# yanivw12/gs2mesh

Measured on AMD Instinct MI355X. Metric: stereo-pair renders/sec + TSDF Mvoxel-updates/sec, higher is better.
Workload: dtype f32

## Files before the change

gs2mesh_amd/csrc/tsdf_kernels.h:

```cpp
#pragma once
#include "tsdf_common.h"


GS2M_DEVICE void tsdf_cam_point(const TsdfFrame& f, float p0, float p1, float p2, float& pc0, float& pc1, float& pc2) {
    pc0 = f.E[0] * p0 + f.E[1] * p1 + f.E[2] * p2 + f.E[3] * 1.f;
    pc1 = f.E[4] * p0 + f.E[5] * p1 + f.E[6] * p2 + f.E[7] * 1.f;
    pc2 = f.E[8] * p0 + f.E[9] * p1 + f.E[10] * p2 + f.E[11] * 1.f;
}
GS2M_DEVICE void tsdf_z_step(const TsdfFrame& f, float& pc0, float& pc1, float& pc2) {
    pc0 += f.Es02;
    pc1 += f.Es12;
    pc2 += f.Es22;
}
GS2M_DEVICE int tsdf_project(const TsdfFrame& f, float pc0, float pc1, float pc2, int& u, int& v) {
    if (pc2 <= 0) return -1;
    const float u_f = pc0 * f.fx_f / pc2 + f.cx_f + 0.5f;
    const float v_f = pc1 * f.fy_f / pc2 + f.cy_f + 0.5f;
    if (!(u_f >= 0.0001f && u_f < f.safe_w && v_f >= 0.0001f && v_f < f.safe_h)) return -1;
    u = (int)u_f;
    v = (int)v_f;
    return v * f.W + u;
}
GS2M_DEVICE float tsdf_distance_multiplier(const TsdfFrame& f, int u, int v) {
    const float xx = (u - f.cx_f) * f.fx_inv_f;
    const float yy = (v - f.cy_f) * f.fy_inv_f;
    return sqrtf(xx * xx + yy * yy + 1.0f);
}
GS2M_DEVICE float tsdf_read_depth(const TsdfFrame& f, const float* __restrict__ depth, const unsigned char* __restrict__ mask, size_t pix) {
    float d = depth[pix];
    if (f.use_mask && mask[pix] == 0) d = d * 0.0f;
    return d;
}
GS2M_DEVICE float tsdf_convert_depth(const TsdfFrame& f, float d) {
    if (f.use_min && d < f.min_depth_f) d = 0.0f;
    if (f.depth_scale_f != 1.0f) d /= f.depth_scale_f;
    if (d >= f.depth_trunc_up_f) d = 0.0f;
    return d;
}
GS2M_DEVICE bool tsdf_decide(const TsdfFrame& f, float d, float zc, float mult, float& tnew) {
    const float sdf = (d - zc) * mult;
    tnew = fminf(1.0f, sdf * f.sdf_trunc_inv_f);
    return d > 0.0f && sdf > -f.sdf_trunc_f;
}
GS2M_DEVICE unsigned tsdf_gather_rgb(const unsigned char* __restrict__ color, int pix, int last_pix) {
    const unsigned char* c = color + 3 * (size_t)pix;
    return pix < last_pix ? gs2m_load_u32_unaligned(c) : ((unsigned)c[0] | ((unsigned)c[1] << 8) | ((unsigned)c[2] << 16));
}
GS2M_DEVICE void tsdf_update_mean(float& t, float& w, float tnew) {
    t = (t * w + tnew) / (w + 1.0f);
    w = w + 1.0f;
}
GS2M_DEVICE void tsdf_update_rgb(unsigned& c0, unsigned& c1, unsigned& c2, unsigned rgbp) {
    c0 += rgbp & 0xffu;
    c1 += (rgbp >> 8) & 0xffu;
    c2 += (rgbp >> 16) & 0xffu;
}
GS2M_DEVICE float tsdf_block_centres(const TsdfFrame& f, unsigned long long key, int tid, float* s_p0, float* s_p1) {
    int bx, by, bz;
    tsdf_unpack_key(key, bx, by, bz);
    const double ox = (double)bx * f.unit_length, oy = (double)by * f.unit_length, oz = (double)bz * f.unit_length;
    if (tid < 16) s_p0[tid] = (float)(f.half_voxel_length_f + f.voxel_length_f * tid + ox);
    else if (tid < 32) s_p1[tid - 16] = (float)(f.half_voxel_length_f + f.voxel_length_f * (tid - 16) + oy);
    return (float)(f.half_voxel_length_f + oz);
}

GS2M_DEVICE unsigned tsdf_find_or_insert(const TsdfVolume& V, unsigned long long key, int bx, int by, int bz) {
    const unsigned mask = V.hash_cap - 1u;
    unsigned h = tsdf_hash(key) & mask;
    for (unsigned probe = 0; probe < V.hash_cap; ++probe, h = (h + 1u) & mask) {
        unsigned long long k = V.hash_keys[h];
        if (k == key) return h;
        if (k == GS2M_TSDF_EMPTY) {
            const unsigned long long prev = atomicCAS(&V.hash_keys[h], GS2M_TSDF_EMPTY, key);
            if (prev == GS2M_TSDF_EMPTY) {
                const unsigned slot = atomicAdd(&V.counters[0], 1u);
                if (slot < V.max_blocks) {
                    V.block_keys[3 * (size_t)slot] = bx;
                    V.block_keys[3 * (size_t)slot + 1] = by;
                    V.block_keys[3 * (size_t)slot + 2] = bz;
                    V.hash_vals[h] = (int)slot;
                } else {
                    atomicOr(&V.counters[2], 1u);
                }
                return h;
            }
            if (prev == key) return h;
        }
    }
    atomicOr(&V.counters[2], 2u);
    return 0xffffffffu;
}

GS2M_DEVICE int tsdf_lookup(const TsdfVolume& V, unsigned long long key) {
    const unsigned mask = V.hash_cap - 1u;
    unsigned h = tsdf_hash(key) & mask;
    for (unsigned probe = 0; probe < V.hash_cap; ++probe, h = (h + 1u) & mask) {
        const unsigned long long k = V.hash_keys[h];
        if (k == key) return V.hash_vals[h];
        if (k == GS2M_TSDF_EMPTY) return -1;
    }
    return -1;
}

struct TouchStage {
    int lo[3][64];
    int hi[3][64];
};

GS2M_DEVICE int wave_min_i(int v) {
#pragma unroll
    for (int m = 32; m > 0; m >>= 1) {
        const int o = gs2m_shfl_xor(v, m);
        v = o < v ? o : v;
    }
    return v;
}
GS2M_DEVICE int wave_max_i(int v) {
#pragma unroll
    for (int m = 32; m > 0; m >>= 1) {
        const int o = gs2m_shfl_xor(v, m);
        v = o > v ? o : v;
    }
    return v;
}

GS2M_DEVICE void tsdf_touch_body(const TsdfVolume& V, const TsdfFrame& f, const float* __restrict__ depth,
                                 const unsigned char* __restrict__ mask, TouchStage* stage_all, int batch_bit) {
    const int lane = (int)(threadIdx.x & 63u);
    TouchStage* stg = &stage_all[threadIdx.x >> 6];
    const int idx = (int)(blockIdx.x * 256u + threadIdx.x);
    int lo[3] = {0x7fffffff, 0x7fffffff, 0x7fffffff}, hi[3] = {-0x7fffffff, -0x7fffffff, -0x7fffffff};
    bool valid = false;
    if (idx < f.nx * f.ny) {
        const int i = (idx / f.nx) * f.stride;
        const int j = (idx % f.nx) * f.stride;
        const float p = tsdf_convert_depth(f, tsdf_read_depth(f, depth, mask, (size_t)i * f.W + j));
        if (p > 0.0f) {
            valid = true;
            const double z = (double)p;
            const double x = (j - f.cx) * z / f.fx;
            const double y = (i - f.cy) * z / f.fy;
#pragma unroll
            for (int r = 0; r < 3; ++r) {
                const double pw = f.pose[4 * r + 0] * x + f.pose[4 * r + 1] * y + f.pose[4 * r + 2] * z + f.pose[4 * r + 3] * 1.0;
                lo[r] = (int)floor((pw - f.sdf_trunc) / f.unit_length);
                hi[r] = (int)floor((pw + f.sdf_trunc) / f.unit_length);
            }
        }
    }
    if (gs2m_ballot(valid ? 1 : 0) == 0ull) return;
    int wlo[3], whi[3];
#pragma unroll
    for (int r = 0; r < 3; ++r) {
        wlo[r] = wave_min_i(lo[r]);
        whi[r] = wave_max_i(hi[r]);
    }
    bool same = lane > 0 && valid;
#pragma unroll
    for (int r = 0; r < 3; ++r) {
        const int plo = gs2m_shfl_up(lo[r], 1), phi = gs2m_shfl_up(hi[r], 1);
        same = same && plo == lo[r] && phi == hi[r];
    }
    const bool pvalid = gs2m_shfl_up(valid ? 1 : 0, 1) != 0;
    const bool keep = valid && !(same && pvalid);
    const unsigned long long kept = gs2m_ballot(keep ? 1 : 0);
    const int n_keep = gs2m_popc64(kept);
    if (keep) {
        const int slot = gs2m_popc64(kept & ((1ull << lane) - 1ull));
#pragma unroll
        for (int r = 0; r < 3; ++r) {
            stg->lo[r][slot] = lo[r];
            stg->hi[r][slot] = hi[r];
        }
    }
    gs2m_wave_sync();
    const long long total_ll = ((long long)whi[0] - wlo[0] + 1) * ((long long)whi[1] - wlo[1] + 1) *
                               ((long long)whi[2] - wlo[2] + 1);
    if (total_ll > (1ll << 24)) {
        if (lane == 0) atomicOr(&V.counters[2], 4u);
        return;
    }
    const int ny = whi[1] - wlo[1] + 1, nz = whi[2] - wlo[2] + 1;
    const int nyz = ny * nz;
    const int total = (int)total_ll;
    for (int base = 0; base < total; base += 64) {
        const int c = base + lane;
        if (c >= total) continue;
        const int cx = c / nyz, rem = c - cx * nyz;
        const int cy = rem / nz;
        const int bx = wlo[0] + cx, by = wlo[1] + cy, bz = wlo[2] + (rem - cy * nz);
        int in_any = 0;
#pragma unroll 4
        for (int k = 0; k < n_keep; ++k)
            in_any |= (int)(bx >= stg->lo[0][k]) & (int)(bx <= stg->hi[0][k]) & (int)(by >= stg->lo[1][k]) &
                      (int)(by <= stg->hi[1][k]) & (int)(bz >= stg->lo[2][k]) & (int)(bz <= stg->hi[2][k]);
        const bool inside = in_any != 0;
        if (!inside) continue;
        if (!tsdf_key_in_range(bx, by, bz)) {
            atomicOr(&V.counters[2], 4u);
            continue;
        }
        const unsigned h = tsdf_find_or_insert(V, tsdf_pack_key(bx, by, bz), bx, by, bz);
        if (h == 0xffffffffu) continue;
        if (batch_bit < 0) {
            if (V.stamp[h] != f.frame_id) V.stamp[h] = f.frame_id;
        } else {
            const unsigned long long bit = 1ull << batch_bit;
            if (!(V.fmask[h] & bit)) atomicOr(&V.fmask[h], bit);
        }
    }
}

GS2M_KERNEL void __launch_bounds__(256)
k_tsdf_touch(TsdfVolume V, TsdfFrame f, const float* __restrict__ depth, const unsigned char* __restrict__ mask) {
    __shared__ TouchStage stage_all[4];
    tsdf_touch_body(V, f, depth, mask, stage_all, -1);
}

GS2M_KERNEL void __launch_bounds__(256)
k_tsdf_touch_batch(TsdfVolume V, const TsdfBatchFrame* __restrict__ frames) {
    __shared__ TouchStage stage_all[4];
    const TsdfBatchFrame& bf = frames[blockIdx.y];
    tsdf_touch_body(V, bf.f, bf.depth, bf.mask, stage_all, (int)blockIdx.y);
}


GS2M_KERNEL void __launch_bounds__(1024)
k_tsdf_compact(TsdfVolume V, unsigned frame_id) {
    __shared__ unsigned wave_cnt[16];
    __shared__ unsigned wg_base;
    const int tid = (int)threadIdx.x, lane = tid & 63, wave = tid >> 6;
    const unsigned h = blockIdx.x * 1024u + (unsigned)tid;
    const bool t = h < V.hash_cap && (frame_id ? V.stamp[h] == frame_id : V.fmask[h] != 0ull);
    const unsigned long long m = gs2m_ballot(t ? 1 : 0);
    if (lane == 0) wave_cnt[wave] = (unsigned)gs2m_popc64(m);
    __syncthreads();
    if (tid == 0) {
        unsigned s = 0;
        for (int k = 0; k < 16; ++k) {
            const unsigned c = wave_cnt[k];
            wave_cnt[k] = s;
            s += c;
        }
        wg_base = s ? atomicAdd(&V.counters[1], s) : 0u;
    }
    __syncthreads();
    if (t) {
        const unsigned rank = (unsigned)gs2m_popc64(m & ((1ull << lane) - 1ull));
        V.touched[wg_base + wave_cnt[wave] + rank] = h;
    }
}

GS2M_KERNEL void __launch_bounds__(256)
k_tsdf_integrate(TsdfVolume V, TsdfFrame f, const float* __restrict__ depth, const unsigned char* __restrict__ color,
                 const unsigned char* __restrict__ mask) {
    __shared__ float s_p0[16], s_p1[16];
    const int tid = (int)threadIdx.x;
    const int lane = tid & 63, wave = tid >> 6;
    const int lz = lane >> 4, lx = (lane >> 2) & 3, ly = lane & 3;
    const unsigned n_touched = V.counters[1];
    const int last_pix = f.W * f.H - 1;
    for (unsigned it = blockIdx.x; it < n_touched; it += gridDim.x) {
        const unsigned h = V.touched[it];
        const unsigned long long key = V.hash_keys[h];
        const int slot = V.hash_vals[h];
        if (slot < 0) continue;
        __syncthreads();
        const float p2 = tsdf_block_centres(f, key, tid, s_p0, s_p1);
        __syncthreads();
        float* bt = V.tsdf + (size_t)slot * GS2M_TSDF_VOX;
        float* bw = V.weight + (size_t)slot * GS2M_TSDF_VOX;
        unsigned* bc = V.rgb + (size_t)slot * 3 * GS2M_TSDF_VOX;
#pragma unroll 1
        for (int g = 0; g < 4; ++g) {
            int pix[4], vi[4];
            float zc[4], mult[4], d[4], tnew[4];
            const int z0 = g * 4;
#pragma unroll
            for (int k = 0; k < 4; ++k) {
                const int mb = g * 16 + wave * 4 + k;
                const int x = wave * 4 + lx, y = k * 4 + ly;
                vi[k] = mb * 64 + lane;
                float pc0, pc1, pc2;
                tsdf_cam_point(f, s_p0[x], s_p1[y], p2, pc0, pc1, pc2);
                for (int s = 0; s < z0; ++s) tsdf_z_step(f, pc0, pc1, pc2);
#pragma unroll
                for (int s = 0; s < 3; ++s) {
                    if (s < lz) tsdf_z_step(f, pc0, pc1, pc2);
                }
                int u = 0, v = 0;
                pix[k] = tsdf_project(f, pc0, pc1, pc2, u, v);
                zc[k] = pc2;
                mult[k] = pix[k] >= 0 ? tsdf_distance_multiplier(f, u, v) : 0.0f;
            }
#pragma unroll
            for (int k = 0; k < 4; ++k)
                d[k] = pix[k] >= 0 ? tsdf_convert_depth(f, tsdf_read_depth(f, depth, mask, (size_t)pix[k])) : 0.0f;
            bool upd[4];
#pragma unroll
            for (int k = 0; k < 4; ++k) {
                const bool hit = tsdf_decide(f, d[k], zc[k], mult[k], tnew[k]);
                upd[k] = pix[k] >= 0 && hit;
            }
            float w[4], t[4];
            unsigned c0[4], c1[4], c2[4], rgbp[4];
#pragma unroll
            for (int k = 0; k < 4; ++k) {
                if (upd[k]) {
                    w[k] = bw[vi[k]];
                    t[k] = bt[vi[k]];
                    if (V.has_color) {
                        c0[k] = bc[vi[k]];
                        c1[k] = bc[GS2M_TSDF_VOX + vi[k]];
                        c2[k] = bc[2 * GS2M_TSDF_VOX + vi[k]];
                        rgbp[k] = tsdf_gather_rgb(color, pix[k], last_pix);
                    }
                }
            }
#pragma unroll
            for (int k = 0; k < 4; ++k) {
                if (upd[k]) {
                    tsdf_update_mean(t[k], w[k], tnew[k]);
                    bt[vi[k]] = t[k];
                    if (V.has_color) {
                        tsdf_update_rgb(c0[k], c1[k], c2[k], rgbp[k]);
                        bc[vi[k]] = c0[k];
                        bc[GS2M_TSDF_VOX + vi[k]] = c1[k];
                        bc[2 * GS2M_TSDF_VOX + vi[k]] = c2[k];
                    }
                    bw[vi[k]] = w[k];
                }
            }
        }
    }
    if (blockIdx.x == 0 && tid == 0) V.totals[0] += n_touched;
}

GS2M_KERNEL void __launch_bounds__(256)
k_tsdf_integrate_batch(TsdfVolume V, const TsdfBatchFrame* __restrict__ frames) {
    __shared__ float s_p0[16], s_p1[16];
    const int tid = (int)threadIdx.x;
    const int lane = tid & 63, wave = tid >> 6;
    const int lz = lane >> 4, lx = (lane >> 2) & 3, ly = lane & 3;
    __shared__ unsigned s_it;
    const unsigned n_touched = V.counters[1] * 4u;
    const TsdfFrame& f0 = frames[0].f;
    for (;;) {
        __syncthreads();
        if (tid == 0) s_it = atomicAdd(&V.counters[3], 1u);
        __syncthreads();
        const unsigned it = s_it;
        if (it >= n_touched) break;
        const int xq = (int)(it & 3u);
        const unsigned h = V.touched[it >> 2];
        const unsigned long long key = V.hash_keys[h];
        const int slot = V.hash_vals[h];
        const unsigned long long fm = V.fmask[h];
        if (slot < 0) continue;
        const float p2 = tsdf_block_centres(f0, key, tid, s_p0, s_p1);
        __syncthreads();
        const float p0 = s_p0[4 * xq + lx], p1 = s_p1[4 * wave + ly];
        const int vi0 = (xq * 4 + wave) * 64 + lane;
        constexpr int VS = 16 * 64;
        float* bt = V.tsdf + (size_t)slot * GS2M_TSDF_VOX;
        float* bw = V.weight + (size_t)slot * GS2M_TSDF_VOX;
        unsigned* bc = V.rgb + (size_t)slot * 3 * GS2M_TSDF_VOX;
        float w[4], t[4];
        unsigned c0[4], c1[4], c2[4];
#pragma unroll
        for (int j = 0; j < 4; ++j) {
            w[j] = bw[vi0 + VS * j];
            t[j] = bt[vi0 + VS * j];
            c0[j] = c1[j] = c2[j] = 0u;
            if (V.has_color) {
                c0[j] = bc[vi0 + VS * j];
                c1[j] = bc[GS2M_TSDF_VOX + vi0 + VS * j];
                c2[j] = bc[2 * GS2M_TSDF_VOX + vi0 + VS * j];
            }
        }
        struct Probe {
            int fi;
            unsigned uv[4];
            float zc0;
            float d[4];
        };
        constexpr unsigned NO_PIXEL = 0xffffffffu;
        auto probe = [&](const int fi, Probe& P) __attribute__((always_inline)) {
            const TsdfBatchFrame& bf = frames[fi];
            const TsdfFrame& f = bf.f;
            const float* __restrict__ depth = bf.depth;
            const unsigned char* __restrict__ mask = bf.mask;
            P.fi = fi;
            float pc0, pc1, pc2;
            tsdf_cam_point(f, p0, p1, p2, pc0, pc1, pc2);
#pragma unroll
            for (int s = 0; s < 3; ++s) {
                if (s < lz) tsdf_z_step(f, pc0, pc1, pc2);
            }
            P.zc0 = pc2;
            int pix[4];
#pragma unroll
            for (int j = 0; j < 4; ++j) {
                int u = 0, v = 0;
                pix[j] = tsdf_project(f, pc0, pc1, pc2, u, v);
                P.uv[j] = pix[j] >= 0 ? ((unsigned)u | ((unsigned)v << 16)) : NO_PIXEL;
#pragma unroll
                for (int s = 0; s < 4; ++s) tsdf_z_step(f, pc0, pc1, pc2);
            }
#pragma unroll
            for (int j = 0; j < 4; ++j)
                P.d[j] = pix[j] >= 0 ? tsdf_read_depth(f, depth, mask, (size_t)pix[j]) : 0.0f;
        };
        auto apply = [&](Probe& P) __attribute__((always_inline)) {
            const TsdfBatchFrame& bf = frames[P.fi];
            const TsdfFrame& f = bf.f;
            const unsigned char* __restrict__ color = bf.color;
            const int last_pix = f.W * f.H - 1;
            unsigned rgbp[4];
            bool upd[4];
            float tnew[4];
            float zx = 0.0f, zy = 0.0f, zc = P.zc0;
#pragma unroll
            for (int j = 0; j < 4; ++j) {
                upd[j] = false;
                tnew[j] = 0.0f;
                rgbp[j] = 0u;
                const bool seen = P.uv[j] != NO_PIXEL;
                const float zcj = zc;
#pragma unroll
                for (int s = 0; s < 4; ++s) tsdf_z_step(f, zx, zy, zc);
                float dd = P.d[j];
                if (seen) dd = tsdf_convert_depth(f, dd);
                if (seen && dd > 0.0f) {
                    const int u = (int)(P.uv[j] & 0xffffu), v = (int)(P.uv[j] >> 16);
                    const float mult = tsdf_distance_multiplier(f, u, v);
                    upd[j] = tsdf_decide(f, dd, zcj, mult, tnew[j]);
                    if (upd[j] && V.has_color) rgbp[j] = tsdf_gather_rgb(color, v * f.W + u, last_pix);
                }
            }
#pragma unroll
            for (int j = 0; j < 4; ++j) {
                if (upd[j]) {
                    tsdf_update_mean(t[j], w[j], tnew[j]);
                    tsdf_update_rgb(c0[j], c1[j], c2[j], rgbp[j]);
                }
            }
        };
        unsigned long long todo = fm;
        Probe A, B;
        if (todo != 0ull) {
            probe(__ffsll(todo) - 1, A);
            todo &= todo - 1ull;
            while (todo != 0ull) {
                probe(__ffsll(todo) - 1, B);
                todo &= todo - 1ull;
                apply(A);
                if (todo == 0ull) {
                    A = B;
                    break;
                }
                probe(__ffsll(todo) - 1, A);
                todo &= todo - 1ull;
                apply(B);
                if (todo == 0ull) break;
            }
            apply(A);
        }
#pragma unroll
        for (int j = 0; j < 4; ++j) {
            bw[vi0 + VS * j] = w[j];
            bt[vi0 + VS * j] = t[j];
            if (V.has_color) {
                bc[vi0 + VS * j] = c0[j];
                bc[GS2M_TSDF_VOX + vi0 + VS * j] = c1[j];
                bc[2 * GS2M_TSDF_VOX + vi0 + VS * j] = c2[j];
            }
        }
        if (tid == 0 && xq == 0) atomicAdd(&V.totals[0], (unsigned long long)gs2m_popc64(fm));
    }
}

GS2M_KERNEL void __launch_bounds__(256)
k_tsdf_clear_fmask(TsdfVolume V) {
    const unsigned n = V.counters[1];
    for (unsigned i = blockIdx.x * 256u + threadIdx.x; i < n; i += gridDim.x * 256u) V.fmask[V.touched[i]] = 0ull;
}

GS2M_KERNEL void __launch_bounds__(256)
k_tsdf_clear_used(TsdfVolume V) {
    unsigned n = V.counters[0];
    if (n > V.max_blocks) n = V.max_blocks;
    const float4 z = {0.f, 0.f, 0.f, 0.f};
    for (unsigned slot = blockIdx.x; slot < n; slot += gridDim.x) {
        float4* t4 = reinterpret_cast<float4*>(V.tsdf + (size_t)slot * GS2M_TSDF_VOX);
        float4* w4 = reinterpret_cast<float4*>(V.weight + (size_t)slot * GS2M_TSDF_VOX);
        for (int i = (int)threadIdx.x; i < GS2M_TSDF_VOX / 4; i += 256) {
            t4[i] = z;
            w4[i] = z;
        }
        if (V.has_color) {
            float4* c4 = reinterpret_cast<float4*>(V.rgb + (size_t)slot * 3 * GS2M_TSDF_VOX);
            for (int i = (int)threadIdx.x; i < 3 * GS2M_TSDF_VOX / 4; i += 256) c4[i] = z;
        }
        if (threadIdx.x == 0) V.halo[slot] = 0;
    }
}

GS2M_KERNEL void __launch_bounds__(256)
k_tsdf_clear_from(TsdfVolume V, unsigned first) {
    unsigned n = V.counters[0];
    if (n > V.max_blocks) n = V.max_blocks;
    const float4 z = {0.f, 0.f, 0.f, 0.f};
    for (unsigned slot = first + blockIdx.x; slot < n; slot += gridDim.x) {
        float4* t4 = reinterpret_cast<float4*>(V.tsdf + (size_t)slot * GS2M_TSDF_VOX);
        float4* w4 = reinterpret_cast<float4*>(V.weight + (size_t)slot * GS2M_TSDF_VOX);
        for (int i = (int)threadIdx.x; i < GS2M_TSDF_VOX / 4; i += 256) {
            t4[i] = z;
            w4[i] = z;
        }
        if (V.has_color) {
            float4* c4 = reinterpret_cast<float4*>(V.rgb + (size_t)slot * 3 * GS2M_TSDF_VOX);
            for (int i = (int)threadIdx.x; i < 3 * GS2M_TSDF_VOX / 4; i += 256) c4[i] = z;
        }
        if (threadIdx.x == 0) V.halo[slot] = 0;
    }
}

GS2M_KERNEL void __launch_bounds__(256)
k_tsdf_clear_gap(TsdfVolume V, unsigned upto) {
    unsigned first = V.counters[0];
    if (upto > V.max_blocks) upto = V.max_blocks;
    const float4 z = {0.f, 0.f, 0.f, 0.f};
    for (unsigned slot = first + blockIdx.x; slot < upto; slot += gridDim.x) {
        float4* t4 = reinterpret_cast<float4*>(V.tsdf + (size_t)slot * GS2M_TSDF_VOX);
        float4* w4 = reinterpret_cast<float4*>(V.weight + (size_t)slot * GS2M_TSDF_VOX);
        for (int i = (int)threadIdx.x; i < GS2M_TSDF_VOX / 4; i += 256) {
            t4[i] = z;
            w4[i] = z;
        }
        if (V.has_color) {
            float4* c4 = reinterpret_cast<float4*>(V.rgb + (size_t)slot * 3 * GS2M_TSDF_VOX);
            for (int i = (int)threadIdx.x; i < 3 * GS2M_TSDF_VOX / 4; i += 256) c4[i] = z;
        }
        if (threadIdx.x == 0) V.halo[slot] = 0;
    }
}

#define GS2M_XF_SUM_F32 0
#define GS2M_XF_RAW_F32 1
#define GS2M_XF_SUM_PACKED 2
template <int FORM>
GS2M_KERNEL void __launch_bounds__(256)
k_tsdf_pack(TsdfVolume V, const int* __restrict__ keys, float* __restrict__ buf, long long* __restrict__ ibuf) {
    const int tid = (int)threadIdx.x;
    const size_t b = blockIdx.x;
    const int bx = keys[3 * b], by = keys[3 * b + 1], bz = keys[3 * b + 2];
    int slot = tsdf_key_in_range(bx, by, bz) ? tsdf_lookup(V, tsdf_pack_key(bx, by, bz)) : -1;
    if (slot >= 0 && FORM != GS2M_XF_RAW_F32 && V.halo[slot]) slot = -1;
    float* o = buf + b * (FORM == GS2M_XF_SUM_PACKED ? 1 : 5) * GS2M_TSDF_VOX;
    for (int i = tid; i < GS2M_TSDF_VOX; i += 256) {
        float w = 0.f, t = 0.f;
        unsigned c0 = 0u, c1 = 0u, c2 = 0u;
        if (slot >= 0) {
            w = V.weight[(size_t)slot * GS2M_TSDF_VOX + i];
            t = V.tsdf[(size_t)slot * GS2M_TSDF_VOX + i];
            if (FORM != GS2M_XF_RAW_F32) t = t * w;
            if (V.has_color) {
                c0 = V.rgb[(size_t)slot * 3 * GS2M_TSDF_VOX + i];
                c1 = V.rgb[(size_t)slot * 3 * GS2M_TSDF_VOX + GS2M_TSDF_VOX + i];
                c2 = V.rgb[(size_t)slot * 3 * GS2M_TSDF_VOX + 2 * GS2M_TSDF_VOX + i];
            }
        }
        o[i] = t;
        if (FORM == GS2M_XF_SUM_PACKED) {
            if (w > 1023.0f || ((c0 | c1 | c2) >> 18) != 0u) atomicOr(&V.counters[2], 8u);
            ibuf[b * GS2M_TSDF_VOX + i] = (long long)((unsigned long long)(unsigned)w | ((unsigned long long)c0 << 10) |
                                                      ((unsigned long long)c1 << 28) | ((unsigned long long)c2 << 46));
        } else {
            o[GS2M_TSDF_VOX + i] = w;
            o[2 * GS2M_TSDF_VOX + i] = (float)c0;
            o[3 * GS2M_TSDF_VOX + i] = (float)c1;
            o[4 * GS2M_TSDF_VOX + i] = (float)c2;
        }
    }
}

template <int FORM>
GS2M_KERNEL void __launch_bounds__(256)
k_tsdf_unpack(TsdfVolume V, const int* __restrict__ keys, const float* __restrict__ buf, const long long* __restrict__ ibuf,
              int halo) {
    __shared__ int s_slot;
    const int tid = (int)threadIdx.x;
    const size_t b = blockIdx.x;
    if (tid == 0) {
        const int bx = keys[3 * b], by = keys[3 * b + 1], bz = keys[3 * b + 2];
        int slot = -1;
        if (tsdf_key_in_range(bx, by, bz)) {
            const unsigned h = tsdf_find_or_insert(V, tsdf_pack_key(bx, by, bz), bx, by, bz);
            if (h != 0xffffffffu) slot = V.hash_vals[h];
        } else {
            atomicOr(&V.counters[2], 4u);
        }
        if (slot >= 0) V.halo[slot] = (unsigned char)(halo ? 1 : 0);
        s_slot = slot;
    }
    __syncthreads();
    const int slot = s_slot;
    if (slot < 0) return;
    const float* in = buf + b * (FORM == GS2M_XF_SUM_PACKED ? 1 : 5) * GS2M_TSDF_VOX;
    for (int i = tid; i < GS2M_TSDF_VOX; i += 256) {
        float w;
        unsigned c0, c1, c2;
        if (FORM == GS2M_XF_SUM_PACKED) {
            const unsigned long long p = (unsigned long long)ibuf[b * GS2M_TSDF_VOX + i];
            w = (float)(unsigned)(p & 0x3ffull);
            c0 = (unsigned)((p >> 10) & 0x3ffffull);
            c1 = (unsigned)((p >> 28) & 0x3ffffull);
            c2 = (unsigned)(p >> 46);
        } else {
            w = in[GS2M_TSDF_VOX + i];
            c0 = (unsigned)in[2 * GS2M_TSDF_VOX + i];
            c1 = (unsigned)in[3 * GS2M_TSDF_VOX + i];
            c2 = (unsigned)in[4 * GS2M_TSDF_VOX + i];
        }
        V.weight[(size_t)slot * GS2M_TSDF_VOX + i] = w;
        V.tsdf[(size_t)slot * GS2M_TSDF_VOX + i] = FORM == GS2M_XF_RAW_F32 ? in[i] : (w > 0.f ? in[i] / w : 0.f);
        if (V.has_color) {
            V.rgb[(size_t)slot * 3 * GS2M_TSDF_VOX + i] = c0;
            V.rgb[(size_t)slot * 3 * GS2M_TSDF_VOX + GS2M_TSDF_VOX + i] = c1;
            V.rgb[(size_t)slot * 3 * GS2M_TSDF_VOX + 2 * GS2M_TSDF_VOX + i] = c2;
        }
    }
}

GS2M_KERNEL void __launch_bounds__(256)
k_tsdf_owned_keys(TsdfVolume V, unsigned n, int* __restrict__ keys) {
    const unsigned s = blockIdx.x * 256u + threadIdx.x;
    if (s >= n) return;
    const bool h = V.halo[s] != 0;
    const int sentinel = GS2M_TSDF_KEY_BIAS - 1;
    keys[3 * (size_t)s] = h ? sentinel : V.block_keys[3 * (size_t)s];
    keys[3 * (size_t)s + 1] = h ? sentinel : V.block_keys[3 * (size_t)s + 1];
    keys[3 * (size_t)s + 2] = h ? sentinel : V.block_keys[3 * (size_t)s + 2];
}

#define GS2M_TSDF_MAP_HEADER 32
GS2M_DEVICE void tsdf_put_u32(unsigned char* p, unsigned v) {
    p[0] = (unsigned char)(v & 255u);
    p[1] = (unsigned char)((v >> 8) & 255u);
    p[2] = (unsigned char)((v >> 16) & 255u);
    p[3] = (unsigned char)(v >> 24);
}
GS2M_KERNEL void __launch_bounds__(256)
k_tsdf_block_map(TsdfVolume V, int lox, int loy, int loz, int dx, int dy, int dz, unsigned char* __restrict__ cells, unsigned n_cells,
                 unsigned flags, unsigned win_hash, int rank, unsigned frames_local, unsigned frames_base) {
    unsigned n = V.counters[0];
    if (n > V.max_blocks) n = V.max_blocks;
    unsigned char* hdr = cells + n_cells;
    if (blockIdx.x == 0 && threadIdx.x == 0) {
        const unsigned ov = V.counters[2];
        for (int b = 0; b < 4; ++b) hdr[1 + b] = (unsigned char)((ov >> b) & 1u);
        hdr[5] = (unsigned char)(flags & 1u);
        hdr[6] = (unsigned char)((flags >> 1) & 1u);
        tsdf_put_u32(hdr + 8, V.max_blocks);
        tsdf_put_u32(hdr + 12, ~V.max_blocks);
        tsdf_put_u32(hdr + 16, win_hash);
        tsdf_put_u32(hdr + 20, ~win_hash);
        tsdf_put_u32(hdr + GS2M_TSDF_MAP_HEADER + 8 * rank, frames_local);
        tsdf_put_u32(hdr + GS2M_TSDF_MAP_HEADER + 8 * rank + 4, frames_base);
    }
    for (unsigned s = blockIdx.x * 256u + threadIdx.x; s < n; s += gridDim.x * 256u) {
        if (V.halo[s]) continue;
        const int bx = V.block_keys[3 * (size_t)s] - lox, by = V.block_keys[3 * (size_t)s + 1] - loy, bz = V.block_keys[3 * (size_t)s + 2] - loz;
        if (bx < 0 || by < 0 || bz < 0 || bx >= dx || by >= dy || bz >= dz) {
            hdr[0] = 1;
            continue;
        }
        cells[((size_t)bx * (unsigned)dy + (unsigned)by) * (unsigned)dz + (unsigned)bz] = 1;
    }
}

GS2M_KERNEL void __launch_bounds__(1024)
k_tsdf_map_keys(int lox, int loy, int loz, int dy, int dz, unsigned char* __restrict__ cells, unsigned n_cells, int* __restrict__ keys,
                unsigned max_keys) {
    __shared__ unsigned wave_sum[16];
    const int tid = (int)threadIdx.x, lane = tid & 63, wave = tid >> 6;
    const unsigned per = ((n_cells + 1023u) / 1024u + 15u) & ~15u;
    const unsigned c0 = (unsigned)tid * per < n_cells ? (unsigned)tid * per : n_cells;
    const unsigned c1 = c0 + per < n_cells ? c0 + per : n_cells;
    unsigned cnt = 0;
    for (unsigned c = c0; c < c1; c += 16u) {
        if (c + 16u <= c1) {
            const uint4 v = *reinterpret_cast<const uint4*>(cells + c);
            const unsigned t = (v.x & 0x01010101u) + (v.y & 0x01010101u) + (v.z & 0x01010101u) + (v.w & 0x01010101u);
            cnt += (t & 255u) + ((t >> 8) & 255u) + ((t >> 16) & 255u) + (t >> 24);
        } else {
            for (unsigned k = c; k < c1; ++k) cnt += cells[k] ? 1u : 0u;
        }
    }
    unsigned inc = cnt;
    for (int d = 1; d < 64; d <<= 1) {
        const unsigned o = gs2m_shfl_up(inc, d);
        if (lane >= d) inc += o;
    }
    if (lane == 63) wave_sum[wave] = inc;
    __syncthreads();
    unsigned base = 0;
    for (int k = 0; k < wave; ++k) base += wave_sum[k];
    unsigned pos = base + inc - cnt;
    if (tid == 1023) tsdf_put_u32(cells + n_cells + 24, base + inc);
    if (cnt == 0u) return;
    for (unsigned c = c0; c < c1; ++c) {
        if (!cells[c]) continue;
        if (pos < max_keys) {
            const unsigned z = c % (unsigned)dz, xy = c / (unsigned)dz;
            keys[3 * (size_t)pos] = (int)(xy / (unsigned)dy) + lox;
            keys[3 * (size_t)pos + 1] = (int)(xy % (unsigned)dy) + loy;
            keys[3 * (size_t)pos + 2] = (int)z + loz;
        }
        ++pos;
    }
}
```

gs2mesh_amd/csrc/tsdf_kernels.hip:

```cpp
#include "tsdf_kernels.h"
#include "tsdf_extract.h"
#include "mesh_kernels.h"
#include "tsdf_internal.h"
#include <math.h>

void gs2m_launch_tsdf_touch(hipStream_t st, const TsdfVolume& V, const TsdfFrame& f, const float* depth,
                            const unsigned char* mask) {
    const int n = f.nx * f.ny;
    GS2M_LAUNCH(k_tsdf_touch, dim3((n + 255) / 256), dim3(256), 0, st, V, f, depth, mask);
    GS2M_LAUNCH(k_tsdf_compact, dim3((V.hash_cap + 1023u) / 1024u), dim3(1024), 0, st, V, f.frame_id);
}
void gs2m_launch_tsdf_integrate(hipStream_t st, int n_wg, const TsdfVolume& V, const TsdfFrame& f,
                                const float* depth, const unsigned char* color, const unsigned char* mask) {
    GS2M_LAUNCH(k_tsdf_integrate, dim3(n_wg), dim3(256), 0, st, V, f, depth, color, mask);
}
void gs2m_launch_tsdf_touch_batch(hipStream_t st, const TsdfVolume& V, const TsdfFrame& f, int n_frames,
                                  const TsdfBatchFrame* frames) {
    const int n = f.nx * f.ny;
    GS2M_LAUNCH(k_tsdf_touch_batch, dim3((n + 255) / 256, n_frames), dim3(256), 0, st, V, frames);
    GS2M_LAUNCH(k_tsdf_compact, dim3((V.hash_cap + 1023u) / 1024u), dim3(1024), 0, st, V, 0u);
}
void gs2m_launch_tsdf_integrate_batch(hipStream_t st, int n_cu, const TsdfVolume& V, const TsdfBatchFrame* frames) {
    GS2M_LAUNCH(k_tsdf_integrate_batch, dim3(n_cu * 6), dim3(256), 0, st, V, frames);
    GS2M_LAUNCH(k_tsdf_clear_fmask, dim3(16), dim3(256), 0, st, V);
}
void gs2m_launch_tsdf_clear_used(hipStream_t st, const TsdfVolume& V) {
    GS2M_LAUNCH(k_tsdf_clear_used, dim3(2048), dim3(256), 0, st, V);
}
void gs2m_launch_tsdf_pack(hipStream_t st, unsigned n, const TsdfVolume& V, const int* keys, int form, float* buf, long long* ibuf) {
    if (form == GS2M_XF_SUM_PACKED) GS2M_LAUNCH(k_tsdf_pack<GS2M_XF_SUM_PACKED>, dim3(n), dim3(256), 0, st, V, keys, buf, ibuf);
    else if (form == GS2M_XF_RAW_F32) GS2M_LAUNCH(k_tsdf_pack<GS2M_XF_RAW_F32>, dim3(n), dim3(256), 0, st, V, keys, buf, ibuf);
    else GS2M_LAUNCH(k_tsdf_pack<GS2M_XF_SUM_F32>, dim3(n), dim3(256), 0, st, V, keys, buf, ibuf);
}
void gs2m_launch_tsdf_unpack(hipStream_t st, unsigned n, const TsdfVolume& V, const int* keys, int form, const float* buf,
                             const long long* ibuf, int halo) {
    if (form == GS2M_XF_SUM_PACKED) GS2M_LAUNCH(k_tsdf_unpack<GS2M_XF_SUM_PACKED>, dim3(n), dim3(256), 0, st, V, keys, buf, ibuf, halo);
    else if (form == GS2M_XF_RAW_F32) GS2M_LAUNCH(k_tsdf_unpack<GS2M_XF_RAW_F32>, dim3(n), dim3(256), 0, st, V, keys, buf, ibuf, halo);
    else GS2M_LAUNCH(k_tsdf_unpack<GS2M_XF_SUM_F32>, dim3(n), dim3(256), 0, st, V, keys, buf, ibuf, halo);
}
void gs2m_launch_tsdf_clear_from(hipStream_t st, const TsdfVolume& V, unsigned first) {
    GS2M_LAUNCH(k_tsdf_clear_from, dim3(1024), dim3(256), 0, st, V, first);
}
void gs2m_launch_tsdf_clear_gap(hipStream_t st, const TsdfVolume& V, unsigned upto) {
    GS2M_LAUNCH(k_tsdf_clear_gap, dim3(256), dim3(256), 0, st, V, upto);
}
void gs2m_launch_tsdf_owned_keys(hipStream_t st, unsigned n, const TsdfVolume& V, int* keys) {
    GS2M_LAUNCH(k_tsdf_owned_keys, dim3((n + 255u) / 256u), dim3(256), 0, st, V, n, keys);
}

void gs2m_launch_tsdf_block_map(hipStream_t st, const TsdfVolume& V, const int* lo, const int* dim, unsigned char* cells, unsigned n_cells,
                                unsigned flags, unsigned win_hash, int rank, unsigned frames_local, unsigned frames_base) {
    const unsigned wg = (V.max_blocks + 255u) / 256u;
    GS2M_LAUNCH(k_tsdf_block_map, dim3(wg < 256u ? (wg ? wg : 1u) : 256u), dim3(256), 0, st, V, lo[0], lo[1], lo[2], dim[0], dim[1], dim[2], cells,
                n_cells, flags, win_hash, rank, frames_local, frames_base);
}
void gs2m_launch_tsdf_map_keys(hipStream_t st, const int* lo, const int* dim, unsigned char* cells, unsigned n_cells, int* keys, unsigned max_keys) {
    GS2M_LAUNCH(k_tsdf_map_keys, dim3(1), dim3(1024), 0, st, lo[0], lo[1], lo[2], dim[1], dim[2], cells, n_cells, keys, max_keys);
}

size_t gs2m_mc_tables_bytes() { return sizeof(McDevTables); }
bool gs2m_mc_tables_fill(void* host_buf) {
    McTables T;
    if (!mc_generate(&T)) return false;
    McDevTables* D = (McDevTables*)host_buf;
    memcpy(D->tri, T.tri, sizeof(T.tri));
    memcpy(D->ntri, T.ntri, sizeof(T.ntri));
    return true;
}
void gs2m_launch_mc_count(hipStream_t st, const TsdfVolume& V, const McDevTables* T, unsigned n_blocks,
                          unsigned* blk_tris, unsigned long long* n_total) {
    GS2M_LAUNCH(k_mc_count, dim3(n_blocks), dim3(256), 0, st, V, T, n_blocks, blk_tris);
    GS2M_LAUNCH(k_mc_scan, dim3(1), dim3(1024), 0, st, blk_tris, n_blocks, n_total);
}
void gs2m_launch_mc_emit(hipStream_t st, const TsdfVolume& V, const McDevTables* T, unsigned n_blocks,
                         const unsigned* blk_off, unsigned long long max_tris, double voxel_length, double unit_length,
                         double* vertices, double* colors, int* edge_index) {
    McGeom G;
    for (int i = 0; i < 8; ++i)
        for (int a = 0; a < 3; ++a) G.corner[i][a] = mc_corner[i][a];
    for (int e = 0; e < 12; ++e)
        for (int a = 0; a < 3; ++a) G.edge[e][a] = mc_edge[e][a];
    GS2M_LAUNCH(k_mc_emit, dim3(n_blocks), dim3(256), 0, st, V, T, G, n_blocks, blk_off, max_tris, voxel_length,
                unit_length, vertices, colors, edge_index);
}

static unsigned grid_for(unsigned n) {
    const unsigned g = (n + 255u) / 256u;
    return g < 1u ? 1u : (g > 4096u ? 4096u : g);
}
void gs2m_launch_scan_u32(hipStream_t st, const unsigned* in, unsigned n, unsigned* out, unsigned* scratch) {
    const unsigned m = (n + GS2M_SCAN_TILE - 1u) / GS2M_SCAN_TILE;
    GS2M_LAUNCH(k_scan_tile_sums, dim3(m), dim3(1024), 0, st, in, n, scratch);
    GS2M_LAUNCH(k_scan_sums, dim3(1), dim3(1024), 0, st, scratch, m, scratch + m);
    GS2M_LAUNCH(k_scan_apply, dim3(m), dim3(1024), 0, st, in, n, scratch, out);
}
void gs2m_launch_mesh_weld_count(hipStream_t st, unsigned n, const int* edge_index, int* mins, unsigned long long* hkeys, unsigned* hfirst,
                                 unsigned cap, unsigned* cell_of, unsigned* flag, unsigned* pos, unsigned* scratch, unsigned* bad) {
    GS2M_LAUNCH(k_mesh_key_min, dim3(grid_for(n)), dim3(256), 0, st, edge_index, n, mins);
    GS2M_LAUNCH(k_mesh_weld_insert, dim3(grid_for(n)), dim3(256), 0, st, edge_index, n, mins, hkeys, hfirst, cap, cell_of, bad);
    GS2M_LAUNCH(k_mesh_weld_flag, dim3(grid_for(n)), dim3(256), 0, st, n, hfirst, cell_of, flag);
    gs2m_launch_scan_u32(st, flag, n, pos, scratch);
}
void gs2m_launch_mesh_weld_emit(hipStream_t st, unsigned n, const unsigned* hfirst, const unsigned* cell_of, const unsigned* pos, const double* verts,
                                const double* cols, const int* edge_index, double* out_v, double* out_c, int* out_e, int* out_tri) {
    GS2M_LAUNCH(k_mesh_weld_emit, dim3(grid_for(n)), dim3(256), 0, st, n, hfirst, cell_of, pos, verts, cols, edge_index, out_v, out_c, out_e,
                out_tri);
}
void gs2m_launch_mesh_cluster(hipStream_t st, const int* tri, unsigned n_tri, unsigned long long* hkeys, unsigned* hval, unsigned cap,
                              unsigned* parent, unsigned* root, unsigned* flag, unsigned* pos, unsigned* scratch, int* labels,
                              unsigned long long* cluster_n) {
    GS2M_LAUNCH(k_mesh_uf_init, dim3(grid_for(n_tri)), dim3(256), 0, st, n_tri, parent);
    GS2M_LAUNCH(k_mesh_uf_edges, dim3(grid_for(n_tri)), dim3(256), 0, st, tri, n_tri, hkeys, hval, cap, parent);
    GS2M_LAUNCH(k_mesh_uf_roots, dim3(grid_for(n_tri)), dim3(256), 0, st, n_tri, parent, root, flag);
    gs2m_launch_scan_u32(st, flag, n_tri, pos, scratch);
    GS2M_LAUNCH(k_mesh_uf_labels, dim3(grid_for(n_tri)), dim3(256), 0, st, n_tri, root, pos, labels, cluster_n);
}
void gs2m_launch_mesh_normals_bucket(hipStream_t st, const double* verts, unsigned nv, const int* tri, unsigned nt, double* tn, unsigned* deg,
                                     unsigned* off, unsigned* fill, unsigned* list, unsigned* owner, unsigned* scratch, unsigned* small) {
    GS2M_LAUNCH(k_mesh_tri_normals, dim3(grid_for(nt)), dim3(256), 0, st, verts, nv, tri, nt, tn, deg, small);
    gs2m_launch_scan_u32(st, deg, nv, off, scratch);
    GS2M_LAUNCH(k_mesh_deg_max, dim3(grid_for(nv)), dim3(256), 0, st, deg, nv, small + 1);
    GS2M_LAUNCH(k_mesh_incidence_scatter, dim3(grid_for(3u * nt)), dim3(256), 0, st, tri, nv, nt, off, fill, list, owner);
}
void gs2m_launch_mesh_bucket_merge(hipStream_t st, unsigned n, unsigned width, const unsigned* off, const unsigned* deg, const unsigned* owner,
                                   const unsigned* src, unsigned* dst) {
    GS2M_LAUNCH(k_mesh_bucket_merge, dim3(grid_for(n)), dim3(256), 0, st, n, width, off, deg, owner, src, dst);
}
void gs2m_launch_mesh_vertex_sum(hipStream_t st, unsigned nv, unsigned nt, const unsigned* off, const unsigned* deg, const unsigned* list,
                                 const double* tn, double* vn) {
    GS2M_LAUNCH(k_mesh_vertex_sum, dim3(grid_for(nv)), dim3(256), 0, st, nv, nt, off, deg, list, tn, vn);
}
```

Measured before the change: 4193.

## Tile TSDF touch into 16x16 pixel blocks with shared-memory block dedup bitmap

Each workgroup now covers a 2D 16x16 tile of subsampled pixels, with each wave taking an 8x8 sub-tile, instead of a linear run of 256 pixels. The four waves' block bounding boxes are merged. When the merged box fits in 1024 cells, touched voxel blocks are first recorded in a shared-memory bitmap and inserted into the hash once per workgroup. The aim is to cut redundant hash find_or_insert probes and atomics for blocks touched by several waves. The cost is two extra __syncthreads, a larger shared allocation, and a fallback path when the union box is too large.

```diff
diff --git a/gs2mesh_amd/csrc/tsdf_kernels.h b/gs2mesh_amd/csrc/tsdf_kernels.h
--- a/gs2mesh_amd/csrc/tsdf_kernels.h
+++ b/gs2mesh_amd/csrc/tsdf_kernels.h
@@ -102,10 +102,17 @@
     return -1;
 }
 
+#define GS2M_TSDF_TOUCH_CELLS 1024
 struct TouchStage {
     int lo[3][64];
     int hi[3][64];
 };
+struct TouchShared {
+    TouchStage stage[4];
+    int wlo[4][3], whi[4][3];
+    int wok[4];
+    unsigned bits[GS2M_TSDF_TOUCH_CELLS / 32];
+};
 
 GS2M_DEVICE int wave_min_i(int v) {
 #pragma unroll
@@ -124,16 +131,32 @@
     return v;
 }
 
+GS2M_DEVICE void tsdf_touch_mark(const TsdfVolume& V, const TsdfFrame& f, int bx, int by, int bz, int batch_bit) {
+    if (!tsdf_key_in_range(bx, by, bz)) {
+        atomicOr(&V.counters[2], 4u);
+        return;
+    }
+    const unsigned h = tsdf_find_or_insert(V, tsdf_pack_key(bx, by, bz), bx, by, bz);
+    if (h == 0xffffffffu) return;
+    if (batch_bit < 0) {
+        if (V.stamp[h] != f.frame_id) V.stamp[h] = f.frame_id;
+    } else {
+        const unsigned long long bit = 1ull << batch_bit;
+        if (!(V.fmask[h] & bit)) atomicOr(&V.fmask[h], bit);
+    }
+}
+
 GS2M_DEVICE void tsdf_touch_body(const TsdfVolume& V, const TsdfFrame& f, const float* __restrict__ depth,
-                                 const unsigned char* __restrict__ mask, TouchStage* stage_all, int batch_bit) {
-    const int lane = (int)(threadIdx.x & 63u);
-    TouchStage* stg = &stage_all[threadIdx.x >> 6];
-    const int idx = (int)(blockIdx.x * 256u + threadIdx.x);
+                                 const unsigned char* __restrict__ mask, TouchShared* sh, int batch_bit) {
+    const int tid = (int)threadIdx.x, lane = tid & 63, wave = tid >> 6;
+    TouchStage* stg = &sh->stage[wave];
+    const int sx = (int)blockIdx.x * 16 + (wave & 1) * 8 + (lane & 7);
+    const int sy = (int)blockIdx.y * 16 + (wave >> 1) * 8 + (lane >> 3);
     int lo[3] = {0x7fffffff, 0x7fffffff, 0x7fffffff}, hi[3] = {-0x7fffffff, -0x7fffffff, -0x7fffffff};
     bool valid = false;
-    if (idx < f.nx * f.ny) {
-        const int i = (idx / f.nx) * f.stride;
-        const int j = (idx % f.nx) * f.stride;
+    if (sx < f.nx && sy < f.ny) {
+        const int i = sy * f.stride;
+        const int j = sx * f.stride;
         const float p = tsdf_convert_depth(f, tsdf_read_depth(f, depth, mask, (size_t)i * f.W + j));
         if (p > 0.0f) {
             valid = true;
@@ -148,80 +171,119 @@
             }
         }
     }
-    if (gs2m_ballot(valid ? 1 : 0) == 0ull) return;
-    int wlo[3], whi[3];
-#pragma unroll
-    for (int r = 0; r < 3; ++r) {
-        wlo[r] = wave_min_i(lo[r]);
-        whi[r] = wave_max_i(hi[r]);
-    }
-    bool same = lane > 0 && valid;
-#pragma unroll
-    for (int r = 0; r < 3; ++r) {
-        const int plo = gs2m_shfl_up(lo[r], 1), phi = gs2m_shfl_up(hi[r], 1);
-        same = same && plo == lo[r] && phi == hi[r];
-    }
-    const bool pvalid = gs2m_shfl_up(valid ? 1 : 0, 1) != 0;
-    const bool keep = valid && !(same && pvalid);
-    const unsigned long long kept = gs2m_ballot(keep ? 1 : 0);
-    const int n_keep = gs2m_popc64(kept);
-    if (keep) {
-        const int slot = gs2m_popc64(kept & ((1ull << lane) - 1ull));
+    const bool any_valid = gs2m_ballot(valid ? 1 : 0) != 0ull;
+    int wlo[3] = {0, 0, 0}, whi[3] = {0, 0, 0};
+    bool wave_ok = false;
+    if (any_valid) {
 #pragma unroll
         for (int r = 0; r < 3; ++r) {
-            stg->lo[r][slot] = lo[r];
-            stg->hi[r][slot] = hi[r];
-        }
-    }
-    gs2m_wave_sync();
-    const long long total_ll = ((long long)whi[0] - wlo[0] + 1) * ((long long)whi[1] - wlo[1] + 1) *
-                               ((long long)whi[2] - wlo[2] + 1);
-    if (total_ll > (1ll << 24)) {
-        if (lane == 0) atomicOr(&V.counters[2], 4u);
-        return;
-    }
-    const int ny = whi[1] - wlo[1] + 1, nz = whi[2] - wlo[2] + 1;
-    const int nyz = ny * nz;
-    const int total = (int)total_ll;
-    for (int base = 0; base < total; base += 64) {
-        const int c = base + lane;
-        if (c >= total) continue;
-        const int cx = c / nyz, rem = c - cx * nyz;
-        const int cy = rem / nz;
-        const int bx = wlo[0] + cx, by = wlo[1] + cy, bz = wlo[2] + (rem - cy * nz);
-        int in_any = 0;
+            wlo[r] = wave_min_i(lo[r]);
+            whi[r] = wave_max_i(hi[r]);
+        }
+        const long long e0 = (long long)whi[0] - wlo[0] + 1, e1 = (long long)whi[1] - wlo[1] + 1, e2 = (long long)whi[2] - wlo[2] + 1;
+        const long long cap = 1ll << 24;
+        wave_ok = e0 <= cap && e1 <= cap && e2 <= cap && e0 * e1 <= cap && e0 * e1 * e2 <= cap;
+        if (!wave_ok && lane == 0) atomicOr(&V.counters[2], 4u);
+    }
+    int n_keep = 0;
+    if (wave_ok) {
+        bool same = lane > 0 && valid;
+#pragma unroll
+        for (int r = 0; r < 3; ++r) {
+            const int plo = gs2m_shfl_up(lo[r], 1), phi = gs2m_shfl_up(hi[r], 1);
+            same = same && plo == lo[r] && phi == hi[r];
+        }
+        const bool pvalid = gs2m_shfl_up(valid ? 1 : 0, 1) != 0;
+        const bool keep = valid && !(same && pvalid);
+        const unsigned long long kept = gs2m_ballot(keep ? 1 : 0);
+        n_keep = gs2m_popc64(kept);
+        if (keep) {
+            const int slot = gs2m_popc64(kept & ((1ull << lane) - 1ull));
+#pragma unroll
+            for (int r = 0; r < 3; ++r) {
+                stg->lo[r][slot] = lo[r];
+                stg->hi[r][slot] = hi[r];
+            }
+        }
+    }
+    if (lane == 0) {
+        sh->wok[wave] = wave_ok ? 1 : 0;
+#pragma unroll
+        for (int r = 0; r < 3; ++r) {
+            sh->wlo[wave][r] = wlo[r];
+            sh->whi[wave][r] = whi[r];
+        }
+    }
+    if (tid < GS2M_TSDF_TOUCH_CELLS / 32) sh->bits[tid] = 0u;
+    __syncthreads();
+    int glo[3] = {0x7fffffff, 0x7fffffff, 0x7fffffff}, ghi[3] = {-0x7fffffff, -0x7fffffff, -0x7fffffff};
+    bool any_ok = false;
+#pragma unroll
+    for (int w = 0; w < 4; ++w) {
+        if (!sh->wok[w]) continue;
+        any_ok = true;
+#pragma unroll
+        for (int r = 0; r < 3; ++r) {
+            glo[r] = sh->wlo[w][r] < glo[r] ? sh->wlo[w][r] : glo[r];
+            ghi[r] = sh->whi[w][r] > ghi[r] ? sh->whi[w][r] : ghi[r];
+        }
+    }
+    bool shared = false;
+    int gny = 1, gnz = 1, gtotal = 0;
+    if (any_ok) {
+        const long long g0 = (long long)ghi[0] - glo[0] + 1, g1 = (long long)ghi[1] - glo[1] + 1, g2 = (long long)ghi[2] - glo[2] + 1;
+        shared = g0 <= GS2M_TSDF_TOUCH_CELLS && g1 <= GS2M_TSDF_TOUCH_CELLS && g2 <= GS2M_TSDF_TOUCH_CELLS &&
+                 g0 * g1 * g2 <= GS2M_TSDF_TOUCH_CELLS;
+        if (shared) {
+            gny = (int)g1;
+            gnz = (int)g2;
+            gtotal = (int)(g0 * g1 * g2);
+        }
+    }
+    if (wave_ok) {
+        const int ny = whi[1] - wlo[1] + 1, nz = whi[2] - wlo[2] + 1;
+        const int nyz = ny * nz;
+        const int total = (whi[0] - wlo[0] + 1) * nyz;
+        for (int base = 0; base < total; base += 64) {
+            const int c = base + lane;
+            if (c >= total) continue;
+            const int cx = c / nyz, rem = c - cx * nyz;
+            const int cy = rem / nz;
+            const int bx = wlo[0] + cx, by = wlo[1] + cy, bz = wlo[2] + (rem - cy * nz);
+            int in_any = 0;
 #pragma unroll 4
-        for (int k = 0; k < n_keep; ++k)
-            in_any |= (int)(bx >= stg->lo[0][k]) & (int)(bx <= stg->hi[0][k]) & (int)(by >= stg->lo[1][k]) &
-                      (int)(by <= stg->hi[1][k]) & (int)(bz >= stg->lo[2][k]) & (int)(bz <= stg->hi[2][k]);
-        const bool inside = in_any != 0;
-        if (!inside) continue;
-        if (!tsdf_key_in_range(bx, by, bz)) {
-            atomicOr(&V.counters[2], 4u);
-            continue;
-        }
-        const unsigned h = tsdf_find_or_insert(V, tsdf_pack_key(bx, by, bz), bx, by, bz);
-        if (h == 0xffffffffu) continue;
-        if (batch_bit < 0) {
-            if (V.stamp[h] != f.frame_id) V.stamp[h] = f.frame_id;
-        } else {
-            const unsigned long long bit = 1ull << batch_bit;
-            if (!(V.fmask[h] & bit)) atomicOr(&V.fmask[h], bit);
-        }
+            for (int k = 0; k < n_keep; ++k)
+                in_any |= (int)(bx >= stg->lo[0][k]) & (int)(bx <= stg->hi[0][k]) & (int)(by >= stg->lo[1][k]) &
+                          (int)(by <= stg->hi[1][k]) & (int)(bz >= stg->lo[2][k]) & (int)(bz <= stg->hi[2][k]);
+            if (in_any == 0) continue;
+            if (shared) {
+                const int cell = ((bx - glo[0]) * gny + (by - glo[1])) * gnz + (bz - glo[2]);
+                atomicOr(&sh->bits[cell >> 5], 1u << (cell & 31));
+            } else {
+                tsdf_touch_mark(V, f, bx, by, bz, batch_bit);
+            }
+        }
+    }
+    __syncthreads();
+    for (int c = tid; c < gtotal; c += 256) {
+        if (!((sh->bits[c >> 5] >> (c & 31)) & 1u)) continue;
+        const int cx = c / (gny * gnz), rem = c - cx * (gny * gnz);
+        const int cy = rem / gnz;
+        tsdf_touch_mark(V, f, glo[0] + cx, glo[1] + cy, glo[2] + (rem - cy * gnz), batch_bit);
     }
 }
 
 GS2M_KERNEL void __launch_bounds__(256)
 k_tsdf_touch(TsdfVolume V, TsdfFrame f, const float* __restrict__ depth, const unsigned char* __restrict__ mask) {
-    __shared__ TouchStage stage_all[4];
-    tsdf_touch_body(V, f, depth, mask, stage_all, -1);
+    __shared__ TouchShared sh;
+    tsdf_touch_body(V, f, depth, mask, &sh, -1);
 }
 
 GS2M_KERNEL void __launch_bounds__(256)
 k_tsdf_touch_batch(TsdfVolume V, const TsdfBatchFrame* __restrict__ frames) {
-    __shared__ TouchStage stage_all[4];
-    const TsdfBatchFrame& bf = frames[blockIdx.y];
-    tsdf_touch_body(V, bf.f, bf.depth, bf.mask, stage_all, (int)blockIdx.y);
+    __shared__ TouchShared sh;
+    const TsdfBatchFrame& bf = frames[blockIdx.z];
+    tsdf_touch_body(V, bf.f, bf.depth, bf.mask, &sh, (int)blockIdx.z);
 }
 
 
diff --git a/gs2mesh_amd/csrc/tsdf_kernels.hip b/gs2mesh_amd/csrc/tsdf_kernels.hip
--- a/gs2mesh_amd/csrc/tsdf_kernels.hip
+++ b/gs2mesh_amd/csrc/tsdf_kernels.hip
@@ -6,8 +6,7 @@
 
 void gs2m_launch_tsdf_touch(hipStream_t st, const TsdfVolume& V, const TsdfFrame& f, const float* depth,
                             const unsigned char* mask) {
-    const int n = f.nx * f.ny;
-    GS2M_LAUNCH(k_tsdf_touch, dim3((n + 255) / 256), dim3(256), 0, st, V, f, depth, mask);
+    GS2M_LAUNCH(k_tsdf_touch, dim3((f.nx + 15) / 16, (f.ny + 15) / 16), dim3(256), 0, st, V, f, depth, mask);
     GS2M_LAUNCH(k_tsdf_compact, dim3((V.hash_cap + 1023u) / 1024u), dim3(1024), 0, st, V, f.frame_id);
 }
 void gs2m_launch_tsdf_integrate(hipStream_t st, int n_wg, const TsdfVolume& V, const TsdfFrame& f,
@@ -16,8 +15,7 @@
 }
 void gs2m_launch_tsdf_touch_batch(hipStream_t st, const TsdfVolume& V, const TsdfFrame& f, int n_frames,
                                   const TsdfBatchFrame* frames) {
-    const int n = f.nx * f.ny;
-    GS2M_LAUNCH(k_tsdf_touch_batch, dim3((n + 255) / 256, n_frames), dim3(256), 0, st, V, frames);
+    GS2M_LAUNCH(k_tsdf_touch_batch, dim3((f.nx + 15) / 16, (f.ny + 15) / 16, n_frames), dim3(256), 0, st, V, frames);
     GS2M_LAUNCH(k_tsdf_compact, dim3((V.hash_cap + 1023u) / 1024u), dim3(1024), 0, st, V, 0u);
 }
 void gs2m_launch_tsdf_integrate_batch(hipStream_t st, int n_cu, const TsdfVolume& V, const TsdfBatchFrame* frames) {
```

After: 4225, median of 6. No clear change (+0.8%).
